# aniketntnu/WordDiffusion

Measured on AMD Instinct MI355X. Metric: denoised 64x256 word images/sec (1000-step DDPM), whole job, higher is better.
Workload: dtype bf16x3; 1 GPU; BASELINE configs[1]: batch 64 per GPU of 64x256 crops = [64,4,8,32] latents, 1000-step DDPM (999 executed steps), base unet.py UNetModel (320 ch, mult (1,1), 4 heads, 339 writers), random-init synthetic weights; variant=base, batch_per_gpu=64, noise_steps=1000, executed_steps_per_image=999, precision=split-bf16 MFMA x3, fp32 accumulate (<=1e-4 of the fp32 reference), output_finite=True

## Files before the change

worddiffusion_amd/csrc/wd_gemmq.hip:

```cpp
#include "wd_gemm_epi.h"
#include "wd_gemm_priv.h"

namespace {

constexpr int QNT = 512;
constexpr int QBM = 64, QBN = 80;
constexpr int QLDE = QBN + 4;
constexpr uint32_t Q_OOB = 0x80000000u;

typedef __attribute__((ext_vector_type(4))) unsigned q_u32x4;

__device__ __forceinline__ int q_lds_off(int row, int ch) { return row * 128 + ((ch ^ ((row >> 1) & 7)) << 4); }

__global__ void __launch_bounds__(QNT, 1) wd_gemmq_kernel(const wd_gemm_args a, const int nbn, const int nbm, const int nchp) {
#if defined(__HIP_DEVICE_COMPILE__)
    extern __shared__ __attribute__((aligned(16))) char smem[];
    const int ntile = nbn * nbm;
    int wg;
    {
        const int bid = blockIdx.x;
        const int q = ntile >> 3, r = ntile & 7, xcd = bid & 7, loc = bid >> 3;
        wg = (xcd < r ? xcd * (q + 1) : r * (q + 1) + (xcd - r) * q) + loc;
    }
    const int bn_i = wg % nbn, bm_i = wg / nbn;
    const int m0 = bm_i * QBM, n0 = bn_i * QBN;
    const int tid = threadIdx.x;
    const int lane = tid & 63;
    const int wave = __builtin_amdgcn_readfirstlane(tid >> 6);
    const int l15 = lane & 15, lq = lane >> 4;

    const int W = a.src[0].ntaps == 9 ? a.slab_rows : 0;
    const int wsh = W ? __builtin_ctz(W) : 0;
    const int ST = (W && a.src[0].hw_src == 4 * a.hw_out) ? 2 : 1;
    const int Ws = W * ST, wss = wsh + ST - 1;
    const int Hs = W ? (a.hw_out >> wsh) * ST : 0;
    const int TR = W ? QBM >> wsh : 0;
    const int NR = W ? (TR - 1) * ST + 3 : 0;
    const int SW = Ws + 2;
    const int bsm = m0 / a.hw_out;
    const int y0 = W ? (m0 - bsm * a.hw_out) >> wsh : 0;

    auto make_srd = [](const void* p) {
        return __builtin_amdgcn_make_buffer_rsrc(const_cast<void*>(p), 0, 0x7FFFFFF0, 0x00020000);
    };
    const __amdgpu_buffer_rsrc_t srd_w_hi = make_srd(a.w_hi), srd_w_lo = make_srd(a.w_lo);

    const int nct = a.n >> 4;
    const uint32_t b_voff = (uint32_t)((n0 >> 4) * 1024 + lane * 16);
    const uint32_t kstep_bytes = (uint32_t)nct * 1024u;
    auto load_b = [&](bf16x8 (&fb)[5][2], const int kabs, const bool live) {
        const uint32_t so = live ? (uint32_t)kabs * kstep_bytes : 0u;
        const uint32_t vo = live ? b_voff : Q_OOB;
#pragma unroll
        for (int t = 0; t < 5; ++t)
#pragma unroll
            for (int p = 0; p < 2; ++p)
                fb[t][p] = __builtin_bit_cast(bf16x8, __builtin_amdgcn_raw_buffer_load_b128(p ? srd_w_lo : srd_w_hi, vo + t * 1024, so, 0));
    };
    f32x4 acc[4][5];
#pragma unroll
    for (int i = 0; i < 4; ++i)
#pragma unroll
        for (int t = 0; t < 5; ++t)
#pragma unroll
            for (int r = 0; r < 4; ++r) acc[i][t][r] = 0.0f;
    auto mfma_step = [&](const char* base, const int cpl, const int (&rb)[4], const int shift0, const int lm, const int half,
                         const bf16x8 (&fb)[5][2], const int skip) {
        const int ach = half * 4 + lq;
        const int shift = shift0 + lm * l15 - l15;
        bf16x8 xa[2][2];
        {
            const int ao = q_lds_off(rb[0] + shift + l15, ach);
            xa[0][0] = *reinterpret_cast<const bf16x8*>(base + ao);
            xa[0][1] = *reinterpret_cast<const bf16x8*>(base + cpl + ao);
        }
#pragma unroll
        for (int i = 0; i < 4; ++i) {
            if (i < 3) {
                const int ao = q_lds_off(rb[i + 1] + shift + l15, ach);
                xa[(i + 1) & 1][0] = *reinterpret_cast<const bf16x8*>(base + ao);
                xa[(i + 1) & 1][1] = *reinterpret_cast<const bf16x8*>(base + cpl + ao);
            }
            if (skip & (1 << i)) continue;
#pragma unroll
            for (int t = 0; t < 5; ++t) {
                acc[i][t] = __builtin_amdgcn_mfma_f32_16x16x32_bf16(xa[i & 1][1], fb[t][0], acc[i][t], 0, 0, 0);
                acc[i][t] = __builtin_amdgcn_mfma_f32_16x16x32_bf16(xa[i & 1][0], fb[t][1], acc[i][t], 0, 0, 0);
                acc[i][t] = __builtin_amdgcn_mfma_f32_16x16x32_bf16(xa[i & 1][0], fb[t][0], acc[i][t], 0, 0, 0);
            }
        }
    };
#ifdef WD_Q_STAMPS
    unsigned long long* qst = (a.dbg & 0x100) && a.ws && blockIdx.x == 0 ? reinterpret_cast<unsigned long long*>(a.ws) + wave * 8 : nullptr;
#define Q_STAMP(i) if (qst && lane == 0) qst[i] = __builtin_amdgcn_s_memtime()
#else
#define Q_STAMP(i)
#endif
    Q_STAMP(0);
    bf16x8 xb[5][2], yb[5][2];
    bool first_pass = true;

    auto run_source = [&](const wd_src& q, const bool conv, const int kbase) {
        const int cpt = q.c >> 6;
        const int slr = conv ? NR * SW : QBM;
        const int cpl = slr * 128, chb = 2 * cpl;
        const int pchunks = min(conv ? 5 : 8, (140 * 1024) / chb);
        const int kpc = conv ? 18 : 2;
        const int ntok = conv ? NR * Ws : QBM;
        const int lm = conv ? ST : 1;
        const __amdgpu_buffer_rsrc_t srd_a_hi = make_srd(q.hi), srd_a_lo = make_srd(q.lo);
        int rb[4];
        int skm0 = 0, skm2 = 0;
#pragma unroll
        for (int i = 0; i < 4; ++i) {
            const int p = 16 * i;
            rb[i] = conv ? ST * (p >> wsh) * SW + ST * (p & (W - 1)) : p;
            if (conv) {
                const int ys = ST * (y0 + (p >> wsh)) - 1;
                if (ys < 0) skm0 |= 1 << i;
                if (ys + 2 >= Hs) skm2 |= 1 << i;
            }
        }
        for (int c_lo = 0; c_lo < cpt; c_lo += pchunks) {
            const int nch = min(pchunks, cpt - c_lo);
            const int nks = kpc * nch;
            if (!first_pass) __syncthreads();
            first_pass = false;
            auto kabs_of = [&](const int c, const int r) {
                return kbase + (conv ? 2 * ((r >> 1) * cpt + c_lo + c) + (r & 1) : 2 * (c_lo + c) + r);
            };
            auto advance = [&](int& c, int& r) {
                if (conv) {
                    r += 8;
                    const bool wrap = r >= 18;
                    r = __builtin_amdgcn_readfirstlane(wrap ? r - 18 : r);
                    c = __builtin_amdgcn_readfirstlane(wrap ? c + 1 : c);
                } else {
                    c += 4;
                }
            };
            auto skip_of = [&](const int r) {
                if (!conv) return 0;
                const int ky = (r >> 1) / 3;
                return __builtin_amdgcn_readfirstlane(ky == 0 ? skm0 : ky == 2 ? skm2 : 0);
            };
            auto shift_of = [&](const int r) {
                if (!conv) return 0;
                const int tap = r >> 1, ky = tap / 3;
                return ky * SW + (tap - 3 * ky);
            };
            int nc = conv ? 0 : wave >> 1, nr = conv ? wave : wave & 1;
            int cc = nc, cr = nr;
            load_b(xb, kabs_of(nc, nr), kpc * nc + nr < nks);
            advance(nc, nr);
            if (conv) {
                for (int i = tid; i < nch * 2 * NR * 2 * 8; i += QNT) {
                    const int pc = i & 7, side = (i >> 3) & 1;
                    int rest = i >> 4;
                    const int ry = rest % NR;
                    rest /= NR;
                    const int pl = rest & 1, ch = rest >> 1;
                    const int row = ry * SW + (side ? SW - 1 : 0);
                    *reinterpret_cast<q_u32x4*>(smem + ch * chb + pl * cpl + row * 128 + pc * 16) = q_u32x4{0u, 0u, 0u, 0u};
                }
            }
            const int nitems = nch * ntok * 8;
            for (int i0 = 0; i0 < nitems; i0 += 8 * QNT) {
                q_u32x4 v[2][8];
                int dst[8];
#pragma unroll
                for (int k = 0; k < 8; ++k) {
                    const int i = i0 + k * QNT + tid;
                    const int pc = i & 7;
                    const int rest = i >> 3;
                    const int chl = rest / ntok, tq = rest - chl * ntok;
                    int grow, srow;
                    bool ok = i < nitems;
                    if (conv) {
                        const int ry = tq >> wss, x = tq & (Ws - 1);
                        const int gy = ST * y0 - 1 + ry;
                        ok = ok && gy >= 0 && gy < Hs;
                        grow = bsm * q.hw_src + gy * Ws + x;
                        srow = ry * SW + x + 1;
                    } else {
                        grow = m0 + tq;
                        srow = tq;
                    }
                    const uint32_t vo = ok ? (uint32_t)grow * (uint32_t)(q.ld * 2) + (uint32_t)((c_lo + chl) * 128 + pc * 16) : Q_OOB;
                    v[0][k] = __builtin_amdgcn_raw_buffer_load_b128(srd_a_hi, vo, 0, 0);
                    v[1][k] = __builtin_amdgcn_raw_buffer_load_b128(srd_a_lo, vo, 0, 0);
                    dst[k] = i < nitems ? chl * chb + q_lds_off(srow, pc) : -1;
                }
#pragma unroll
                for (int k = 0; k < 8; ++k)
                    if (dst[k] >= 0) {
                        *reinterpret_cast<q_u32x4*>(smem + dst[k]) = v[0][k];
                        *reinterpret_cast<q_u32x4*>(smem + dst[k] + cpl) = v[1][k];
                    }
            }
            __syncthreads();
            Q_STAMP(1);
            for (int ks = wave; ks < nks; ks += 16) {
                load_b(yb, kabs_of(nc, nr), kpc * nc + nr < nks);
                advance(nc, nr);
                __builtin_amdgcn_sched_barrier(0);
                mfma_step(smem + cc * chb, cpl, rb, shift_of(cr), lm, cr & 1, xb, skip_of(cr));
                __builtin_amdgcn_sched_barrier(0);
                advance(cc, cr);
                load_b(xb, kabs_of(nc, nr), kpc * nc + nr < nks);
                advance(nc, nr);
                __builtin_amdgcn_sched_barrier(0);
                if (kpc * cc + cr < nks) mfma_step(smem + cc * chb, cpl, rb, shift_of(cr), lm, cr & 1, yb, skip_of(cr));
                __builtin_amdgcn_sched_barrier(0);
                advance(cc, cr);
            }
        }
    };
    const bool conv0 = a.src[0].ntaps == 9;
    run_source(a.src[0], conv0, 0);
    if (a.nsrc > 1) run_source(a.src[1], false, 2 * a.src[0].ntaps * (a.src[0].c >> 6));

    Q_STAMP(4);
    __syncthreads();
    Q_STAMP(5);
    constexpr int IMG = QBM * QLDE;
    constexpr int CLD = QBM + 4;
    constexpr int PIMG = QBN * CLD;
    float* res = reinterpret_cast<float*>(smem);
    float* part = res + IMG;
    auto pcol = [&](float* b, const int i, const int t) -> f32x4* {
        return reinterpret_cast<f32x4*>(b + (t * 16 + l15) * CLD + i * 16 + 4 * lq);
    };
    if (wave >= 4) {
        float* b = part + (wave - 4) * PIMG;
#pragma unroll
        for (int i = 0; i < 4; ++i)
#pragma unroll
            for (int t = 0; t < 5; ++t) *pcol(b, i, t) = acc[i][t];
    }
    __syncthreads();
    if (wave < 4) {
        float* b = part + wave * PIMG;
#pragma unroll
        for (int i = 0; i < 4; ++i)
#pragma unroll
            for (int t = 0; t < 5; ++t) {
                acc[i][t] += *pcol(b, i, t);
                *pcol(b, i, t) = acc[i][t];
            }
    }
    __syncthreads();
    for (int e = tid; e < QBN * (QBM / 4); e += QNT) {
        const int col = e >> 4, r4 = (e & 15) * 4;
        const float* p = part + col * CLD + r4;
        f32x4 v = *reinterpret_cast<const f32x4*>(p);
        v += *reinterpret_cast<const f32x4*>(p + PIMG);
        v += *reinterpret_cast<const f32x4*>(p + 2 * PIMG);
        v += *reinterpret_cast<const f32x4*>(p + 3 * PIMG);
#pragma unroll
        for (int r = 0; r < 4; ++r) res[(r4 + r) * QLDE + col] = v[r];
    }
    __syncthreads();
    float* buf = res;
    Q_STAMP(6);
    if (a.gn_gamma) wd_gn_tile<QBN, QNT, false>(a, buf, buf + IMG, m0, n0, tid);
    else wd_epilogue_tail<QBM, QBN, QNT>(a, buf, m0, n0, tid, 0);
    Q_STAMP(7);
#endif
}

}

bool wd_gemmq_applies(const wd_gemm_args& a) {
    const int W = a.slab_rows;
    if (!(a.w_layout == 3 && a.tile == 64080 && !a.a32 && !a.ln_gamma && a.npass == 3 && a.ksplit <= 1 && a.m % 64 == 0 && a.n % QBN == 0 &&
          a.act == WD_ACT_NONE && !a.resid_rows && a.nsrc >= 1 && a.nsrc <= 2))
        return false;
    for (int s = 0; s < a.nsrc; ++s) {
        const wd_src& q = a.src[s];
        if (!q.hi || !q.lo || q.c % 64 || (q.ld & 7)) return false;
        const bool conv = s == 0 && q.ntaps == 9 && q.gather && a.hw_out == 64 &&
                          (((W == 16 || W == 32) && q.hw_src == 64) || (W == 16 && q.hw_src == 256));
        const bool ident = q.ntaps == 1 && !q.gather;
        if (!conv && !ident) return false;
    }
    return true;
}

int wd_gemmq_launch(const wd_gemm_args& a, hipStream_t st) {
    const int loop_smem = 140 * 1024;
    const int red_smem = (QBM * QLDE + 4 * QBN * (QBM + 4)) * 4 + WD_STAT_SCRATCH;
    const int smem = loop_smem > red_smem ? loop_smem : red_smem;
    const int nchp = 0;
    static int attr_max = 0;
    if (smem > attr_max) {
        if (hipFuncSetAttribute(reinterpret_cast<const void*>(&wd_gemmq_kernel), hipFuncAttributeMaxDynamicSharedMemorySize, smem) != hipSuccess)
            return WD_ELAUNCH;
        attr_max = smem;
    }
    const int nbn = a.n / QBN, nbm = a.m / QBM;
    {
        WdLaunchScope scope(WD_CLS_GEMM_Q, st, 2.0 * (double)a.m * (double)a.n * (double)a.ktot);
        hipLaunchKernelGGL(wd_gemmq_kernel, dim3(nbn * nbm), dim3(QNT), smem, st, a, nbn, nbm, nchp);
    }
    return wd_check_launch();
}
```

worddiffusion_amd/csrc/wd_ff.hip:

```cpp
#include "wd_gemm_epi.h"

namespace {

constexpr int FNT = 512;
constexpr int FBM = 64;
constexpr int FC = 320;
constexpr int FCH = 128;
constexpr int FRING = 6;
constexpr int F_MAX_INNER = 2048;
constexpr int FGRP = 30;
constexpr uint32_t F_OOB = 0x80000000u;

typedef __attribute__((ext_vector_type(4))) unsigned f_u32x4;

__device__ __forceinline__ int f_lds_off(int row, int ch) { return row * 128 + ((ch ^ ((row >> 1) & 7)) << 4); }

template <int NPASS, bool PROJ, bool FRONT>
__global__ void __launch_bounds__(FNT, 1) wd_ff_kernel(const wd_ff_args a) {
#if defined(__HIP_DEVICE_COMPILE__)
    static_assert(!FRONT || (NPASS == 3 && PROJ), "the transformer front needs split-bf16 operands and the proj_out tail");
    constexpr int NPL = (NPASS == 1) ? 1 : 2;
    constexpr int SLAB = 2 * FBM * 128;
    constexpr int A_BYTES = 5 * SLAB;
    constexpr int H_BYTES = 2 * SLAB;
    extern __shared__ __attribute__((aligned(16))) char smem[];
    char* s_a = smem;
    char* s_h = smem + A_BYTES;
    float* s_b1 = reinterpret_cast<float*>(smem + A_BYTES + 2 * H_BYTES);

    const int m0 = blockIdx.x * FBM;
    const int tid = threadIdx.x;
    const int lane = tid & 63;
    const int wave = __builtin_amdgcn_readfirstlane(tid >> 6);
    const int kh = wave >> 2, cg = wave & 3;
    const int l15 = lane & 15, lq = lane >> 4;
    const int nchunk = a.inner / FCH;

    auto make_srd = [](const wd_bf16* p) {
        return __builtin_amdgcn_make_buffer_rsrc(const_cast<wd_bf16*>(p), 0, 0x7FFFFFF0, 0x00020000);
    };
    const __amdgpu_buffer_rsrc_t srd1_hi = make_srd(a.w1_hi), srd1_lo = make_srd(a.w1_lo ? a.w1_lo : a.w1_hi);
    const __amdgpu_buffer_rsrc_t srd2_hi = make_srd(a.w2_hi), srd2_lo = make_srd(a.w2_lo ? a.w2_lo : a.w2_hi);
    const __amdgpu_buffer_rsrc_t srd3_hi = make_srd(PROJ ? a.w3_hi : a.w2_hi), srd3_lo = make_srd(PROJ ? (a.w3_lo ? a.w3_lo : a.w3_hi) : a.w2_hi);
    const uint32_t lane16 = lane * 16;
    const int nct1 = (2 * a.inner) >> 4;

    bf16x8 ring[FRING][NPL];
    auto issue = [&](const int slot, const int g, const int j) {
        const bool live = j < nchunk;
        const uint32_t vo = live ? lane16 : F_OOB;
        if (PROJ && g < FRING) {
            const uint32_t so3 = (uint32_t)(((2 * (g / 5) + kh) * (FC / 16) + 5 * cg + g % 5) * 1024);
            const uint32_t so1 = (uint32_t)(((g >> 1) * nct1 + 2 * (j * 8 + wave) + (g & 1)) * 1024);
            const uint32_t so = live ? so1 : so3;
#pragma unroll
            for (int p = 0; p < NPL; ++p) {
                const __amdgpu_buffer_rsrc_t srd = live ? (p ? srd1_lo : srd1_hi) : (p ? srd3_lo : srd3_hi);
                ring[slot][p] = __builtin_bit_cast(bf16x8, __builtin_amdgcn_raw_buffer_load_b128(srd, lane16, so, 0));
            }
        } else if (g < 20) {
            const uint32_t so = (uint32_t)(((g >> 1) * nct1 + 2 * (j * 8 + wave) + (g & 1)) * 1024);
#pragma unroll
            for (int p = 0; p < NPL; ++p)
                ring[slot][p] = __builtin_bit_cast(bf16x8, __builtin_amdgcn_raw_buffer_load_b128(p ? srd1_lo : srd1_hi, vo, live ? so : 0u, 0));
        } else {
            const int q = (g - 20) / 5, t = (g - 20) % 5;
            const uint32_t so = (uint32_t)(((4 * j + 2 * kh + q) * (FC / 16) + 5 * cg + t) * 1024);
#pragma unroll
            for (int p = 0; p < NPL; ++p)
                ring[slot][p] = __builtin_bit_cast(bf16x8, __builtin_amdgcn_raw_buffer_load_b128(p ? srd2_lo : srd2_hi, vo, live ? so : 0u, 0));
        }
    };
    f32x4 acc2[4][5];
    bf16x8 xa[4][NPL];
    auto read_frags = [&](const char* slab_base, const int half) {
        const int ch = half * 4 + lq;
#pragma unroll
        for (int i = 0; i < 4; ++i) {
            const int ao = f_lds_off(i * 16 + l15, ch);
#pragma unroll
            for (int p = 0; p < NPL; ++p) xa[i][p] = *reinterpret_cast<const bf16x8*>(slab_base + p * (FBM * 128) + ao);
        }
    };
    auto mfma12 = [&](f32x4 (&acc)[4], const bf16x8 (&w)[NPL]) {
#pragma unroll
        for (int i = 0; i < 4; ++i) {
            if (NPL == 2) {
                acc[i] = __builtin_amdgcn_mfma_f32_16x16x32_bf16(xa[i][NPL - 1], w[0], acc[i], 0, 0, 0);
                acc[i] = __builtin_amdgcn_mfma_f32_16x16x32_bf16(xa[i][0], w[NPL - 1], acc[i], 0, 0, 0);
            }
            acc[i] = __builtin_amdgcn_mfma_f32_16x16x32_bf16(xa[i][0], w[0], acc[i], 0, 0, 0);
        }
    };
    constexpr int LDE = FC + 4;
    float* ep = reinterpret_cast<float*>(smem);
    auto ksum_to_image = [&]() {
        for (int hh = 0; hh < 2; ++hh) {
            if (kh == hh) {
#pragma unroll
                for (int i = 0; i < 4; ++i)
#pragma unroll
                    for (int t = 0; t < 5; ++t)
#pragma unroll
                        for (int r = 0; r < 4; ++r) {
                            float* pe = ep + (i * 16 + 4 * lq + r) * LDE + cg * 80 + t * 16 + l15;
                            *pe = (hh == 0) ? acc2[i][t][r] : *pe + acc2[i][t][r];
                        }
            }
            __syncthreads();
        }
    };

    if constexpr (FRONT) {
        constexpr int SP = 65, PP = 72, KS32 = FC / 32;
        const int b = m0 / a.hw;
        const int HJ = a.heads * a.L;
        char* fr = s_h + 4096;
        float* s_aff = reinterpret_cast<float*>(fr);
        float* sS = reinterpret_cast<float*>(fr);
        wd_bf16* sP = reinterpret_cast<wd_bf16*>(fr + FBM * SP * 4);
        {
            const int ngp = FC / a.gn_pcpg, ratio = a.gn_cpg / a.gn_pcpg;
            for (int c = tid; c < FC; c += FNT) {
                const int g = c / a.gn_cpg;
                double su = 0.0, sq = 0.0;
                for (int k = 0; k < ratio; ++k)
                    for (int ck = 0; ck < a.gn_nchunk; ++ck) {
                        const double* pp = a.gn_part + (((long)b * a.gn_nchunk + ck) * ngp + g * ratio + k) * 2;
                        su += pp[0];
                        sq += pp[1];
                    }
                const double n = (double)a.hw * a.gn_cpg;
                const double mu = su / n;
                double var = sq / n - mu * mu;
                if (var < 0.0) var = 0.0;
                const float rstd = (float)(1.0 / sqrt(var + (double)a.gn_eps));
                const float sc = rstd * a.gn_gamma[c];
                s_aff[2 * c] = sc;
                s_aff[2 * c + 1] = a.gn_beta[c] - (float)mu * sc;
            }
            for (int e = tid; e < FBM * PP; e += FNT) reinterpret_cast<uint32_t*>(sP)[e] = 0u;
        }
        const int arow = tid >> 3, ach = tid & 7;
        float4 xv[5][2];
        {
            const float* xrow = a.x_in + (long)(m0 + arow) * a.x_in_ld + ach * 8;
#pragma unroll
            for (int sl = 0; sl < 5; ++sl) {
                xv[sl][0] = *reinterpret_cast<const float4*>(xrow + sl * 64);
                xv[sl][1] = *reinterpret_cast<const float4*>(xrow + sl * 64 + 4);
            }
        }
        const __amdgpu_buffer_rsrc_t srdp_hi = make_srd(a.pi_hi), srdp_lo = make_srd(a.pi_lo);
        auto issue_pi = [&](const int slot, const int g) {
            const uint32_t so = (uint32_t)(((2 * (g / 5) + kh) * (FC / 16) + 5 * cg + g % 5) * 1024);
#pragma unroll
            for (int p = 0; p < NPL; ++p)
                ring[slot][p] = __builtin_bit_cast(bf16x8, __builtin_amdgcn_raw_buffer_load_b128(p ? srdp_lo : srdp_hi, lane16, so, 0));
        };
#pragma unroll
        for (int g = 0; g < FRING; ++g) issue_pi(g, g);
        __syncthreads();
#pragma unroll
        for (int sl = 0; sl < 5; ++sl) {
            const float4* tab = reinterpret_cast<const float4*>(s_aff + 2 * (sl * 64 + ach * 8));
            const float4 t0 = tab[0], t1 = tab[1], t2 = tab[2], t3 = tab[3];
            const float4 x0 = xv[sl][0], x1 = xv[sl][1];
            float4 y0, y1;
            y0.x = x0.x * t0.x + t0.y; y0.y = x0.y * t0.z + t0.w; y0.z = x0.z * t1.x + t1.y; y0.w = x0.w * t1.z + t1.w;
            y1.x = x1.x * t2.x + t2.y; y1.y = x1.y * t2.z + t2.w; y1.z = x1.z * t3.x + t3.y; y1.w = x1.w * t3.z + t3.w;
            uint2 h0, l0, h1, l1;
            wd_split4(y0, h0, l0);
            wd_split4(y1, h1, l1);
            char* dst = s_a + sl * SLAB + f_lds_off(arow, ach);
            *reinterpret_cast<f_u32x4*>(dst) = f_u32x4{h0.x, h0.y, h1.x, h1.y};
            *reinterpret_cast<f_u32x4*>(dst + FBM * 128) = f_u32x4{l0.x, l0.y, l1.x, l1.y};
        }
        __syncthreads();
#pragma unroll
        for (int i = 0; i < 4; ++i)
#pragma unroll
            for (int t = 0; t < 5; ++t)
#pragma unroll
                for (int r = 0; r < 4; ++r) acc2[i][t][r] = 0.0f;
#pragma unroll
        for (int g = 0; g < 25; ++g) {
            const int q = g / 5, t = g % 5;
            if (t == 0) read_frags(s_a + q * SLAB, kh);
            {
                f32x4 col[4] = {acc2[0][t], acc2[1][t], acc2[2][t], acc2[3][t]};
                mfma12(col, ring[g % FRING]);
#pragma unroll
                for (int i = 0; i < 4; ++i) acc2[i][t] = col[i];
            }
            if (g + FRING < 25) issue_pi(g % FRING, g + FRING);
            __builtin_amdgcn_sched_barrier(0);
        }
        __syncthreads();
        ksum_to_image();
        float4 xr[2][5];
#pragma unroll
        for (int pp = 0; pp < 2; ++pp)
#pragma unroll
            for (int i = 0; i < 5; ++i) {
                const int n = (l15 + 16 * i) * 4, row = wave * 8 + pp * 4 + lq;
                const float4 v = *reinterpret_cast<const float4*>(ep + row * LDE + n);
                const float4 bx = *reinterpret_cast<const float4*>(a.pi_b + n);
                xr[pp][i] = make_float4(v.x + bx.x, v.y + bx.y, v.z + bx.z, v.w + bx.w);
            }
        __syncthreads();
        auto ln_rows = [&](const float* gamma, const float* beta) {
#pragma unroll
            for (int pp = 0; pp < 2; ++pp) {
                const int row = wave * 8 + pp * 4 + lq;
                float s = 0.f;
#pragma unroll
                for (int i = 0; i < 5; ++i) s += (xr[pp][i].x + xr[pp][i].y) + (xr[pp][i].z + xr[pp][i].w);
                const float mean = wd_row16_sum(s) / (float)FC;
                float q = 0.f;
#pragma unroll
                for (int i = 0; i < 5; ++i) {
                    const float a0 = xr[pp][i].x - mean, a1 = xr[pp][i].y - mean, a2 = xr[pp][i].z - mean, a3 = xr[pp][i].w - mean;
                    q += (a0 * a0 + a1 * a1) + (a2 * a2 + a3 * a3);
                }
                const float rstd = 1.0f / sqrtf(wd_row16_sum(q) / (float)FC + a.ln_eps);
#pragma unroll
                for (int i = 0; i < 5; ++i) {
                    const int n = (l15 + 16 * i) * 4;
                    const float4 ga = *reinterpret_cast<const float4*>(gamma + n);
                    const float4 be = *reinterpret_cast<const float4*>(beta + n);
                    const float4 x = xr[pp][i];
                    float4 o;
                    o.x = (x.x - mean) * rstd * ga.x + be.x; o.y = (x.y - mean) * rstd * ga.y + be.y;
                    o.z = (x.z - mean) * rstd * ga.z + be.z; o.w = (x.w - mean) * rstd * ga.w + be.w;
                    uint2 hi, lo;
                    wd_split4(o, hi, lo);
                    char* d = s_a + (n >> 6) * SLAB + f_lds_off(row, (n & 63) >> 3) + (n & 7) * 2;
                    *reinterpret_cast<uint2*>(d) = hi;
                    *reinterpret_cast<uint2*>(d + FBM * 128) = lo;
                }
            }
        };
        const int ht = wave & 3, rp = wave >> 2;
        const long pq = 64L * FC;
#pragma unroll
        for (int ps = 0; ps < 2; ++ps) {
            const wd_bf16* mq = ps == 0 ? a.mq_a : a.mq_b;
            const wd_bf16* mot = ps == 0 ? a.mot_a : a.mot_b;
            const float* xb = ps == 0 ? a.xb_a : a.xb_b;
            ln_rows(a.ln2_gamma, a.ln2_beta);
            __builtin_amdgcn_sched_barrier(0);
            bf16x8 bh[KS32], bl[KS32];
            {
                const __amdgpu_buffer_rsrc_t rq = __builtin_amdgcn_make_buffer_rsrc(const_cast<wd_bf16*>(mq + (long)b * 2 * pq), 0,
                                                                                    (int)(2 * pq * 2), 0x00020000);
                const uint32_t vo = ht * 16 + l15 < HJ ? lane16 : F_OOB;
#pragma unroll
                for (int ks = 0; ks < KS32; ++ks) {
                    bh[ks] = __builtin_bit_cast(bf16x8, __builtin_amdgcn_raw_buffer_load_b128(rq, vo, (uint32_t)((ht * KS32 + ks) << 10), 0));
                    bl[ks] = __builtin_bit_cast(bf16x8, __builtin_amdgcn_raw_buffer_load_b128(rq, vo, (uint32_t)(((ht * KS32 + ks) << 10) + pq * 2), 0));
                }
            }
            __syncthreads();
            if (ht * 16 < HJ) {
                f32x4 a_lh[2], a_hl[2], a_hh[2];
#pragma unroll
                for (int ri = 0; ri < 2; ++ri)
#pragma unroll
                    for (int r = 0; r < 4; ++r) a_lh[ri][r] = a_hl[ri][r] = a_hh[ri][r] = 0.f;
#pragma unroll
                for (int ks = 0; ks < KS32; ++ks)
#pragma unroll
                    for (int ri = 0; ri < 2; ++ri) {
                        const char* ap = s_a + (ks >> 1) * SLAB + f_lds_off((2 * rp + ri) * 16 + l15, (ks & 1) * 4 + lq);
                        const bf16x8 ah = *reinterpret_cast<const bf16x8*>(ap);
                        const bf16x8 al = *reinterpret_cast<const bf16x8*>(ap + FBM * 128);
                        a_lh[ri] = __builtin_amdgcn_mfma_f32_16x16x32_bf16(al, bh[ks], a_lh[ri], 0, 0, 0);
                        a_hl[ri] = __builtin_amdgcn_mfma_f32_16x16x32_bf16(ah, bl[ks], a_hl[ri], 0, 0, 0);
                        a_hh[ri] = __builtin_amdgcn_mfma_f32_16x16x32_bf16(ah, bh[ks], a_hh[ri], 0, 0, 0);
                    }
#pragma unroll
                for (int ri = 0; ri < 2; ++ri)
#pragma unroll
                    for (int r = 0; r < 4; ++r)
                        sS[((2 * rp + ri) * 16 + 4 * lq + r) * SP + ht * 16 + l15] = (a_lh[ri][r] + a_hl[ri][r]) + a_hh[ri][r];
            }
            __builtin_amdgcn_sched_barrier(0);
            bf16x8 mh[2][5], ml[2][5];
            {
                const __amdgpu_buffer_rsrc_t rm = __builtin_amdgcn_make_buffer_rsrc(const_cast<wd_bf16*>(mot + (long)b * 2 * pq), 0,
                                                                                    (int)(2 * pq * 2), 0x00020000);
#pragma unroll
                for (int ks = 0; ks < 2; ++ks) {
                    const uint32_t vo = ks * 32 + lq * 8 < HJ ? lane16 : F_OOB;
#pragma unroll
                    for (int t = 0; t < 5; ++t) {
                        const uint32_t so = (uint32_t)((((5 * cg + t) * 2 + ks) << 10));
                        mh[ks][t] = __builtin_bit_cast(bf16x8, __builtin_amdgcn_raw_buffer_load_b128(rm, vo, so, 0));
                        ml[ks][t] = __builtin_bit_cast(bf16x8, __builtin_amdgcn_raw_buffer_load_b128(rm, vo, so + (uint32_t)(pq * 2), 0));
                    }
                }
            }
            __syncthreads();
            for (int idx = tid; idx < FBM * a.heads; idx += FNT) {
                const int t = idx / a.heads, h = idx - t * a.heads;
                const float* pr = sS + t * SP + h * a.L;
                wd_bf16* ph = sP + t * PP + h * a.L;
                float mx = -3.4e38f;
                for (int j = 0; j < a.L; ++j) mx = fmaxf(mx, pr[j]);
                float sum = 0.f;
                for (int j = 0; j < a.L; ++j) sum += __expf(pr[j] - mx);
                const float inv = __fdividef(1.f, sum);
                for (int j = 0; j < a.L; ++j) {
                    uint32_t hi, lo;
                    wd_split1(__expf(pr[j] - mx) * inv, hi, lo);
                    ph[j] = (wd_bf16)hi;
                    ph[FBM * PP + j] = (wd_bf16)lo;
                }
            }
            __syncthreads();
            {
                f32x4 o[2][5];
#pragma unroll
                for (int ri = 0; ri < 2; ++ri)
#pragma unroll
                    for (int t = 0; t < 5; ++t)
#pragma unroll
                        for (int r = 0; r < 4; ++r) o[ri][t][r] = 0.f;
#pragma unroll
                for (int ks = 0; ks < 2; ++ks)
#pragma unroll
                    for (int ri = 0; ri < 2; ++ri) {
                        const wd_bf16* ap = sP + ((2 * rp + ri) * 16 + l15) * PP + lq * 8 + ks * 32;
                        const bf16x8 ah = *reinterpret_cast<const bf16x8*>(ap);
                        const bf16x8 al = *reinterpret_cast<const bf16x8*>(ap + FBM * PP);
#pragma unroll
                        for (int t = 0; t < 5; ++t) o[ri][t] = __builtin_amdgcn_mfma_f32_16x16x32_bf16(al, mh[ks][t], o[ri][t], 0, 0, 0);
#pragma unroll
                        for (int t = 0; t < 5; ++t) o[ri][t] = __builtin_amdgcn_mfma_f32_16x16x32_bf16(ah, ml[ks][t], o[ri][t], 0, 0, 0);
#pragma unroll
                        for (int t = 0; t < 5; ++t) o[ri][t] = __builtin_amdgcn_mfma_f32_16x16x32_bf16(ah, mh[ks][t], o[ri][t], 0, 0, 0);
                    }
#pragma unroll
                for (int ri = 0; ri < 2; ++ri)
#pragma unroll
                    for (int t = 0; t < 5; ++t)
#pragma unroll
                        for (int r = 0; r < 4; ++r) ep[((2 * rp + ri) * 16 + 4 * lq + r) * LDE + (5 * cg + t) * 16 + l15] = o[ri][t][r];
            }
            __syncthreads();
#pragma unroll
            for (int pp = 0; pp < 2; ++pp)
#pragma unroll
                for (int i = 0; i < 5; ++i) {
                    const int n = (l15 + 16 * i) * 4, row = wave * 8 + pp * 4 + lq;
                    const float4 bi = *reinterpret_cast<const float4*>(xb + n);
                    const float4 at = *reinterpret_cast<const float4*>(ep + row * LDE + n);
                    const float4 x = xr[pp][i];
                    xr[pp][i] = make_float4(at.x + bi.x + x.x, at.y + bi.y + x.y, at.z + bi.z + x.z, at.w + bi.w + x.w);
                }
            __syncthreads();
        }
#pragma unroll
        for (int pp = 0; pp < 2; ++pp)
#pragma unroll
            for (int i = 0; i < 5; ++i)
                *reinterpret_cast<float4*>(a.tok2 + (long)(m0 + wave * 8 + pp * 4 + lq) * FC + (l15 + 16 * i) * 4) = xr[pp][i];
        ln_rows(a.ln3_gamma, a.ln3_beta);
        for (int i = tid; i < 2 * a.inner; i += FNT) s_b1[i] = a.b1 ? a.b1[i] : 0.0f;
        __builtin_amdgcn_sched_barrier(0);
#pragma unroll
        for (int g = 0; g < FRING; ++g) issue(g, g, 0);
    } else {
#pragma unroll
    for (int g = 0; g < FRING; ++g) issue(g, g, 0);

    {
        const __amdgpu_buffer_rsrc_t sx_hi = make_srd(a.x_hi), sx_lo = make_srd(a.x_lo ? a.x_lo : a.x_hi);
        const int arow = tid >> 3, ach = tid & 7;
        const uint32_t vo = (m0 + arow < a.m) ? (uint32_t)(m0 + arow) * (uint32_t)(a.x_ld * 2) + (uint32_t)(ach * 16) : F_OOB;
        f_u32x4 v[5][NPL];
#pragma unroll
        for (int sl = 0; sl < 5; ++sl)
#pragma unroll
            for (int p = 0; p < NPL; ++p) v[sl][p] = __builtin_amdgcn_raw_buffer_load_b128(p ? sx_lo : sx_hi, vo, sl * 128, 0);
        const int dst = f_lds_off(arow, ach);
#pragma unroll
        for (int sl = 0; sl < 5; ++sl)
#pragma unroll
            for (int p = 0; p < NPL; ++p) *reinterpret_cast<f_u32x4*>(s_a + sl * SLAB + p * (FBM * 128) + dst) = v[sl][p];
        for (int i = tid; i < 2 * a.inner; i += FNT) s_b1[i] = a.b1 ? a.b1[i] : 0.0f;
    }
    }
    __syncthreads();

#pragma unroll
    for (int i = 0; i < 4; ++i)
#pragma unroll
        for (int t = 0; t < 5; ++t)
#pragma unroll
            for (int r = 0; r < 4; ++r) acc2[i][t][r] = 0.0f;

    for (int j = 0; j < nchunk; ++j) {
        char* hbuf = s_h + (j & 1) * H_BYTES;
        f32x4 ax[4], ag[4];
#pragma unroll
        for (int i = 0; i < 4; ++i)
#pragma unroll
            for (int r = 0; r < 4; ++r) {
                ax[i][r] = 0.0f;
                ag[i][r] = 0.0f;
            }
#pragma unroll
        for (int g = 0; g < 20; ++g) {
            if ((g & 1) == 0) read_frags(s_a + (g >> 2) * SLAB, (g >> 1) & 1);
            if (g & 1) mfma12(ag, ring[g % FRING]);
            else mfma12(ax, ring[g % FRING]);
            if (g + FRING < FGRP) issue(g % FRING, g + FRING, j);
            else issue(g % FRING, g + FRING - FGRP, j + 1);
            __builtin_amdgcn_sched_barrier(0);
        }
        {
            const int hcol = (j * 8 + wave) * 32 + l15;
            const float bx = s_b1[hcol], bg = s_b1[hcol + 16];
            const int slab = wave >> 2, ch = (wave & 3) * 2 + (l15 >> 3), e = (l15 & 7) * 2;
#pragma unroll
            for (int i = 0; i < 4; ++i)
#pragma unroll
                for (int r = 0; r < 4; ++r) {
                    const float h = (ax[i][r] + bx) * wd_gelu_erf(ag[i][r] + bg);
                    uint32_t hb, lb;
                    wd_split1(h, hb, lb);
                    char* p = hbuf + slab * SLAB + f_lds_off(i * 16 + lq * 4 + r, ch) + e;
                    *reinterpret_cast<unsigned short*>(p) = (unsigned short)hb;
                    if (NPL == 2) *reinterpret_cast<unsigned short*>(p + FBM * 128) = (unsigned short)lb;
                }
        }
        __syncthreads();
#pragma unroll
        for (int g = 20; g < FGRP; ++g) {
            const int q = (g - 20) / 5, t = (g - 20) % 5;
            if (t == 0) read_frags(hbuf + kh * SLAB, q);
            {
                f32x4 col[4] = {acc2[0][t], acc2[1][t], acc2[2][t], acc2[3][t]};
                mfma12(col, ring[g % FRING]);
#pragma unroll
                for (int i = 0; i < 4; ++i) acc2[i][t] = col[i];
            }
            if (g + FRING < FGRP) issue(g % FRING, g + FRING, j);
            else issue(g % FRING, g + FRING - FGRP, j + 1);
            __builtin_amdgcn_sched_barrier(0);
        }
    }

    __syncthreads();
    ksum_to_image();
    wd_gemm_args e = {};
    e.m = a.m;
    e.n = FC;
    e.hw_out = a.hw_out > 0 ? a.hw_out : 1;
    e.act = WD_ACT_NONE;
    e.out_f32 = a.out_f32;
    e.out_ld = a.out_ld;
    e.out_hi = a.out_hi;
    e.out_lo = a.out_lo;
    e.out_pl_ld = a.out_pl_ld;
    e.ksplit = 1;
    e.stat_part = a.stat_part;
    e.stat_cpg = a.stat_cpg;
    if constexpr (!PROJ) {
        e.bias = a.b2;
        e.resid = a.resid;
        e.resid_ld = a.resid_ld;
        wd_epilogue_from_image<FBM, FC, FNT>(e, ep, m0, 0, tid);
    } else {
        constexpr int ROWB = LDE * 4;
        const float* resid = FRONT ? a.tok2 : a.resid;
        const int resid_ld = FRONT ? FC : a.resid_ld;
        if (FRONT) asm volatile("s_waitcnt vmcnt(0)" ::: "memory");
        {
            float4 v[10];
#pragma unroll
            for (int it = 0; it < 10; ++it) {
                const int idx = it * 64 + lane, row = wave * 8 + idx / 80, c = (idx % 80) * 4;
                const int m = m0 + row;
                float4 x = *reinterpret_cast<const float4*>(ep + row * LDE + c);
                if (a.b2) {
                    const float4 q = *reinterpret_cast<const float4*>(a.b2 + c);
                    x.x += q.x; x.y += q.y; x.z += q.z; x.w += q.w;
                }
                if (resid && m < a.m) {
                    const float4 q = *reinterpret_cast<const float4*>(resid + (long)m * resid_ld + c);
                    x.x += q.x; x.y += q.y; x.z += q.z; x.w += q.w;
                }
                v[it] = x;
            }
            asm volatile("s_waitcnt lgkmcnt(0)" ::: "memory");
            __builtin_amdgcn_sched_barrier(0);
#pragma unroll
            for (int it = 0; it < 10; ++it) {
                const int idx = it * 64 + lane, row = wave * 8 + idx / 80, c = (idx % 80) * 4;
                uint2 hh, ll;
                wd_split4(v[it], hh, ll);
                char* rowp = reinterpret_cast<char*>(ep) + row * ROWB;
                *reinterpret_cast<uint2*>(rowp + c * 2) = hh;
                if (NPL == 2) *reinterpret_cast<uint2*>(rowp + 640 + c * 2) = ll;
            }
        }
        __syncthreads();
#pragma unroll
        for (int i = 0; i < 4; ++i)
#pragma unroll
            for (int t = 0; t < 5; ++t)
#pragma unroll
                for (int r = 0; r < 4; ++r) acc2[i][t][r] = 0.0f;
#pragma unroll
        for (int g = 0; g < 25; ++g) {
            const int q = g / 5, t = g % 5;
            if (t == 0) {
                const int ks = 2 * q + kh;
#pragma unroll
                for (int i = 0; i < 4; ++i) {
                    const char* rp = reinterpret_cast<const char*>(ep) + (i * 16 + l15) * ROWB + (ks * 4 + lq) * 16;
#pragma unroll
                    for (int p = 0; p < NPL; ++p) xa[i][p] = *reinterpret_cast<const bf16x8*>(rp + p * 640);
// ... 85 lines not shown
```

Measured before the change: 34.15 images/s.

## Stream identity GEMM A operands from registers and overlap conv LDS fill with MFMA

Identity (1x1) sources no longer stage A tiles through LDS. Each wave loads its A fragments directly from global memory with double-buffered registers, which removes the fill pass and barriers. For the 3x3 conv source, only the first channel chunk is filled before compute starts. The remaining chunks are loaded in small batches interleaved with the first MFMA steps, followed by one barrier. The LDS budget grows to 160KB, and the direct global A loads may be less coalesced and less reused than the shared LDS tile was.

Measured after the change: 34.24 images/s (median of 6 runs). About the same (+0.2%).

```diff
diff --git a/worddiffusion_amd/csrc/wd_gemmq.hip b/worddiffusion_amd/csrc/wd_gemmq.hip
--- a/worddiffusion_amd/csrc/wd_gemmq.hip
+++ b/worddiffusion_amd/csrc/wd_gemmq.hip
@@ -6,6 +6,7 @@
 constexpr int QNT = 512;
 constexpr int QBM = 64, QBN = 80;
 constexpr int QLDE = QBN + 4;
+constexpr int Q_LOOP_SMEM = 160 * 1024;
 constexpr uint32_t Q_OOB = 0x80000000u;
 
 typedef __attribute__((ext_vector_type(4))) unsigned q_u32x4;
@@ -100,125 +101,183 @@
     bf16x8 xb[5][2], yb[5][2];
     bool first_pass = true;
 
-    auto run_source = [&](const wd_src& q, const bool conv, const int kbase) {
+    auto run_ident = [&](const wd_src& q, const int kbase) {
+        const int nks = 2 * (q.c >> 6);
+        const __amdgpu_buffer_rsrc_t srd_a_hi = make_srd(q.hi), srd_a_lo = make_srd(q.lo);
+        const uint32_t rowb = (uint32_t)q.ld * 2u;
+        const uint32_t a_voff = (uint32_t)(m0 + l15) * rowb + (uint32_t)(lq * 16);
+        auto load_a = [&](bf16x8 (&fa)[4][2], const int ks, const bool live) {
+            const uint32_t so = live ? (uint32_t)ks * 64u : 0u;
+#pragma unroll
+            for (int i = 0; i < 4; ++i) {
+                const uint32_t vo = live ? a_voff + (uint32_t)(16 * i) * rowb : Q_OOB;
+#pragma unroll
+                for (int p = 0; p < 2; ++p)
+                    fa[i][p] = __builtin_bit_cast(bf16x8, __builtin_amdgcn_raw_buffer_load_b128(p ? srd_a_lo : srd_a_hi, vo, so, 0));
+            }
+        };
+        auto mfma_regs = [&](const bf16x8 (&fa)[4][2], const bf16x8 (&fb)[5][2]) {
+#pragma unroll
+            for (int i = 0; i < 4; ++i)
+#pragma unroll
+                for (int t = 0; t < 5; ++t) {
+                    acc[i][t] = __builtin_amdgcn_mfma_f32_16x16x32_bf16(fa[i][1], fb[t][0], acc[i][t], 0, 0, 0);
+                    acc[i][t] = __builtin_amdgcn_mfma_f32_16x16x32_bf16(fa[i][0], fb[t][1], acc[i][t], 0, 0, 0);
+                    acc[i][t] = __builtin_amdgcn_mfma_f32_16x16x32_bf16(fa[i][0], fb[t][0], acc[i][t], 0, 0, 0);
+                }
+        };
+        bf16x8 xa[4][2], ya[4][2];
+        load_b(xb, kbase + wave, wave < nks);
+        load_a(xa, wave, wave < nks);
+        for (int ks = wave; ks < nks; ks += 16) {
+            load_b(yb, kbase + ks + 8, ks + 8 < nks);
+            load_a(ya, ks + 8, ks + 8 < nks);
+            __builtin_amdgcn_sched_barrier(0);
+            mfma_regs(xa, xb);
+            __builtin_amdgcn_sched_barrier(0);
+            load_b(xb, kbase + ks + 16, ks + 16 < nks);
+            load_a(xa, ks + 16, ks + 16 < nks);
+            __builtin_amdgcn_sched_barrier(0);
+            if (ks + 8 < nks) mfma_regs(ya, yb);
+            __builtin_amdgcn_sched_barrier(0);
+        }
+    };
+
+    constexpr int QR = 2;
+    auto run_source = [&](const wd_src& q, const int kbase) {
         const int cpt = q.c >> 6;
-        const int slr = conv ? NR * SW : QBM;
-        const int cpl = slr * 128, chb = 2 * cpl;
-        const int pchunks = min(conv ? 5 : 8, (140 * 1024) / chb);
-        const int kpc = conv ? 18 : 2;
-        const int ntok = conv ? NR * Ws : QBM;
-        const int lm = conv ? ST : 1;
+        const int cpl = NR * SW * 128, chb = 2 * cpl;
+        const int pchunks = min(5, Q_LOOP_SMEM / chb);
+        constexpr int kpc = 18;
+        const int ntok = NR * Ws;
         const __amdgpu_buffer_rsrc_t srd_a_hi = make_srd(q.hi), srd_a_lo = make_srd(q.lo);
         int rb[4];
         int skm0 = 0, skm2 = 0;
 #pragma unroll
         for (int i = 0; i < 4; ++i) {
             const int p = 16 * i;
-            rb[i] = conv ? ST * (p >> wsh) * SW + ST * (p & (W - 1)) : p;
-            if (conv) {
-                const int ys = ST * (y0 + (p >> wsh)) - 1;
-                if (ys < 0) skm0 |= 1 << i;
-                if (ys + 2 >= Hs) skm2 |= 1 << i;
-            }
+            rb[i] = ST * (p >> wsh) * SW + ST * (p & (W - 1));
+            const int ys = ST * (y0 + (p >> wsh)) - 1;
+            if (ys < 0) skm0 |= 1 << i;
+            if (ys + 2 >= Hs) skm2 |= 1 << i;
         }
         for (int c_lo = 0; c_lo < cpt; c_lo += pchunks) {
             const int nch = min(pchunks, cpt - c_lo);
             const int nks = kpc * nch;
             if (!first_pass) __syncthreads();
             first_pass = false;
-            auto kabs_of = [&](const int c, const int r) {
-                return kbase + (conv ? 2 * ((r >> 1) * cpt + c_lo + c) + (r & 1) : 2 * (c_lo + c) + r);
-            };
+            auto kabs_of = [&](const int c, const int r) { return kbase + 2 * ((r >> 1) * cpt + c_lo + c) + (r & 1); };
             auto advance = [&](int& c, int& r) {
-                if (conv) {
-                    r += 8;
-                    const bool wrap = r >= 18;
-                    r = __builtin_amdgcn_readfirstlane(wrap ? r - 18 : r);
-                    c = __builtin_amdgcn_readfirstlane(wrap ? c + 1 : c);
-                } else {
-                    c += 4;
-                }
+                r += 8;
+                const bool wrap = r >= 18;
+                r = __builtin_amdgcn_readfirstlane(wrap ? r - 18 : r);
+                c = __builtin_amdgcn_readfirstlane(wrap ? c + 1 : c);
             };
             auto skip_of = [&](const int r) {
-                if (!conv) return 0;
                 const int ky = (r >> 1) / 3;
                 return __builtin_amdgcn_readfirstlane(ky == 0 ? skm0 : ky == 2 ? skm2 : 0);
             };
             auto shift_of = [&](const int r) {
-                if (!conv) return 0;
                 const int tap = r >> 1, ky = tap / 3;
                 return ky * SW + (tap - 3 * ky);
             };
-            int nc = conv ? 0 : wave >> 1, nr = conv ? wave : wave & 1;
+            int nc = 0, nr = wave;
             int cc = nc, cr = nr;
             load_b(xb, kabs_of(nc, nr), kpc * nc + nr < nks);
             advance(nc, nr);
-            if (conv) {
-                for (int i = tid; i < nch * 2 * NR * 2 * 8; i += QNT) {
-                    const int pc = i & 7, side = (i >> 3) & 1;
-                    int rest = i >> 4;
-                    const int ry = rest % NR;
-                    rest /= NR;
-                    const int pl = rest & 1, ch = rest >> 1;
-                    const int row = ry * SW + (side ? SW - 1 : 0);
-                    *reinterpret_cast<q_u32x4*>(smem + ch * chb + pl * cpl + row * 128 + pc * 16) = q_u32x4{0u, 0u, 0u, 0u};
-                }
-            }
-            const int nitems = nch * ntok * 8;
-            for (int i0 = 0; i0 < nitems; i0 += 8 * QNT) {
-                q_u32x4 v[2][8];
-                int dst[8];
-#pragma unroll
-                for (int k = 0; k < 8; ++k) {
+            for (int i = tid; i < nch * 2 * NR * 2 * 8; i += QNT) {
+                const int pc = i & 7, side = (i >> 3) & 1;
+                int rest = i >> 4;
+                const int ry = rest % NR;
+                rest /= NR;
+                const int pl = rest & 1, ch = rest >> 1;
+                const int row = ry * SW + (side ? SW - 1 : 0);
+                *reinterpret_cast<q_u32x4*>(smem + ch * chb + pl * cpl + row * 128 + pc * 16) = q_u32x4{0u, 0u, 0u, 0u};
+            }
+            const int nitems = nch * ntok * 8, n0 = ntok * 8;
+            auto fill_load = [&](q_u32x4 (&v)[2][QR], const int i0, const int iend) {
+#pragma unroll
+                for (int k = 0; k < QR; ++k) {
                     const int i = i0 + k * QNT + tid;
                     const int pc = i & 7;
                     const int rest = i >> 3;
                     const int chl = rest / ntok, tq = rest - chl * ntok;
-                    int grow, srow;
-                    bool ok = i < nitems;
-                    if (conv) {
-                        const int ry = tq >> wss, x = tq & (Ws - 1);
-                        const int gy = ST * y0 - 1 + ry;
-                        ok = ok && gy >= 0 && gy < Hs;
-                        grow = bsm * q.hw_src + gy * Ws + x;
-                        srow = ry * SW + x + 1;
-                    } else {
-                        grow = m0 + tq;
-                        srow = tq;
-                    }
+                    const int ry = tq >> wss, x = tq & (Ws - 1);
+                    const int gy = ST * y0 - 1 + ry;
+                    const bool ok = i < iend && gy >= 0 && gy < Hs;
+                    const int grow = bsm * q.hw_src + gy * Ws + x;
                     const uint32_t vo = ok ? (uint32_t)grow * (uint32_t)(q.ld * 2) + (uint32_t)((c_lo + chl) * 128 + pc * 16) : Q_OOB;
                     v[0][k] = __builtin_amdgcn_raw_buffer_load_b128(srd_a_hi, vo, 0, 0);
                     v[1][k] = __builtin_amdgcn_raw_buffer_load_b128(srd_a_lo, vo, 0, 0);
-                    dst[k] = i < nitems ? chl * chb + q_lds_off(srow, pc) : -1;
                 }
-#pragma unroll
-                for (int k = 0; k < 8; ++k)
-                    if (dst[k] >= 0) {
-                        *reinterpret_cast<q_u32x4*>(smem + dst[k]) = v[0][k];
-                        *reinterpret_cast<q_u32x4*>(smem + dst[k] + cpl) = v[1][k];
+            };
+            auto fill_store = [&](const q_u32x4 (&v)[2][QR], const int i0, const int iend) {
+#pragma unroll
+                for (int k = 0; k < QR; ++k) {
+                    const int i = i0 + k * QNT + tid;
+                    if (i < iend) {
+                        const int pc = i & 7;
+                        const int rest = i >> 3;
+                        const int chl = rest / ntok, tq = rest - chl * ntok;
+                        const int ry = tq >> wss, x = tq & (Ws - 1);
+                        const int dst = chl * chb + q_lds_off(ry * SW + x + 1, pc);
+                        *reinterpret_cast<q_u32x4*>(smem + dst) = v[0][k];
+                        *reinterpret_cast<q_u32x4*>(smem + dst + cpl) = v[1][k];
                     }
+                }
+            };
+            q_u32x4 fv[2][QR];
+            for (int i0 = 0; i0 < n0; i0 += QR * QNT) {
+                fill_load(fv, i0, n0);
+                fill_store(fv, i0, n0);
             }
             __syncthreads();
             Q_STAMP(1);
-            for (int ks = wave; ks < nks; ks += 16) {
+            auto step_x = [&]() {
                 load_b(yb, kabs_of(nc, nr), kpc * nc + nr < nks);
                 advance(nc, nr);
                 __builtin_amdgcn_sched_barrier(0);
-                mfma_step(smem + cc * chb, cpl, rb, shift_of(cr), lm, cr & 1, xb, skip_of(cr));
+                mfma_step(smem + cc * chb, cpl, rb, shift_of(cr), ST, cr & 1, xb, skip_of(cr));
                 __builtin_amdgcn_sched_barrier(0);
                 advance(cc, cr);
+            };
+            auto step_y = [&]() {
                 load_b(xb, kabs_of(nc, nr), kpc * nc + nr < nks);
                 advance(nc, nr);
                 __builtin_amdgcn_sched_barrier(0);
-                if (kpc * cc + cr < nks) mfma_step(smem + cc * chb, cpl, rb, shift_of(cr), lm, cr & 1, yb, skip_of(cr));
+                if (kpc * cc + cr < nks) mfma_step(smem + cc * chb, cpl, rb, shift_of(cr), ST, cr & 1, yb, skip_of(cr));
                 __builtin_amdgcn_sched_barrier(0);
                 advance(cc, cr);
+            };
+            int ks = wave;
+            if (nch > 1) {
+                int i0 = n0;
+                fill_load(fv, i0, nitems);
+                __builtin_amdgcn_sched_barrier(0);
+                step_x();
+                fill_store(fv, i0, nitems);
+                i0 += QR * QNT;
+                fill_load(fv, i0, nitems);
+                __builtin_amdgcn_sched_barrier(0);
+                step_y();
+                fill_store(fv, i0, nitems);
+                for (i0 += QR * QNT; i0 < nitems; i0 += QR * QNT) {
+                    fill_load(fv, i0, nitems);
+                    fill_store(fv, i0, nitems);
+                }
+                __syncthreads();
+                ks += 16;
+            }
+            for (; ks < nks; ks += 16) {
+                step_x();
+                step_y();
             }
         }
     };
     const bool conv0 = a.src[0].ntaps == 9;
-    run_source(a.src[0], conv0, 0);
-    if (a.nsrc > 1) run_source(a.src[1], false, 2 * a.src[0].ntaps * (a.src[0].c >> 6));
+    if (conv0) run_source(a.src[0], 0);
+    else run_ident(a.src[0], 0);
+    if (a.nsrc > 1) run_ident(a.src[1], 2 * a.src[0].ntaps * (a.src[0].c >> 6));
 
     Q_STAMP(4);
     __syncthreads();
@@ -288,7 +347,7 @@
 }
 
 int wd_gemmq_launch(const wd_gemm_args& a, hipStream_t st) {
-    const int loop_smem = 140 * 1024;
+    const int loop_smem = Q_LOOP_SMEM;
     const int red_smem = (QBM * QLDE + 4 * QBN * (QBM + 4)) * 4 + WD_STAT_SCRATCH;
     const int smem = loop_smem > red_smem ? loop_smem : red_smem;
     const int nchp = 0;
```

## Prefetch front-path vectors, GN partials and next-stage weights earlier in fused FF kernel

Applied to the files above, without the earlier changes.

In the transformer-front path of the fused feed-forward kernel, the GroupNorm partial sums, bias/LayerNorm parameter vectors and b1 are now loaded into registers up front and staged into LDS once, instead of being read from global memory inside later loops. The mq weight fragments for each cross-attention pass and the first FF weight ring slots are issued earlier, during the previous stage's MFMA work, so their latency overlaps compute. This raises register pressure and uses more LDS, and it relies on a static LDS map assertion holding.

New measurement: 34.18 images/s before, 34.63 images/s after, median of 6. 1.01x the previous value.

```diff
diff --git a/worddiffusion_amd/csrc/wd_ff.hip b/worddiffusion_amd/csrc/wd_ff.hip
--- a/worddiffusion_amd/csrc/wd_ff.hip
+++ b/worddiffusion_amd/csrc/wd_ff.hip
@@ -119,28 +119,35 @@
         float* s_aff = reinterpret_cast<float*>(fr);
         float* sS = reinterpret_cast<float*>(fr);
         wd_bf16* sP = reinterpret_cast<wd_bf16*>(fr + FBM * SP * 4);
-        {
-            const int ngp = FC / a.gn_pcpg, ratio = a.gn_cpg / a.gn_pcpg;
-            for (int c = tid; c < FC; c += FNT) {
-                const int g = c / a.gn_cpg;
-                double su = 0.0, sq = 0.0;
-                for (int k = 0; k < ratio; ++k)
-                    for (int ck = 0; ck < a.gn_nchunk; ++ck) {
-                        const double* pp = a.gn_part + (((long)b * a.gn_nchunk + ck) * ngp + g * ratio + k) * 2;
-                        su += pp[0];
-                        sq += pp[1];
-                    }
-                const double n = (double)a.hw * a.gn_cpg;
-                const double mu = su / n;
-                double var = sq / n - mu * mu;
-                if (var < 0.0) var = 0.0;
-                const float rstd = (float)(1.0 / sqrt(var + (double)a.gn_eps));
-                const float sc = rstd * a.gn_gamma[c];
-                s_aff[2 * c] = sc;
-                s_aff[2 * c + 1] = a.gn_beta[c] - (float)mu * sc;
-            }
-            for (int e = tid; e < FBM * PP; e += FNT) reinterpret_cast<uint32_t*>(sP)[e] = 0u;
-        }
+        float* s_vec = reinterpret_cast<float*>(s_h + 40960);
+        const float* s_pib = s_vec;
+        const float *s_ln2g = s_vec + FC, *s_ln2b = s_vec + 2 * FC, *s_ln3g = s_vec + 3 * FC, *s_ln3b = s_vec + 4 * FC;
+        const float *s_xba = s_vec + 5 * FC, *s_xbb = s_vec + 6 * FC;
+        constexpr int NVEC = 7, V4 = FC / 4;
+        static_assert(4096 + FBM * SP * 4 + 2 * FBM * PP * 2 <= 40960 && 40960 + NVEC * FC * 4 <= 2 * H_BYTES, "front LDS map");
+        auto vec_src = [&](const int i) {
+            const int v = i / V4;
+            const float* p = v == 0 ? a.pi_b : v == 1 ? a.ln2_gamma : v == 2 ? a.ln2_beta : v == 3 ? a.ln3_gamma : v == 4 ? a.ln3_beta
+                           : v == 5 ? a.xb_a : a.xb_b;
+            return reinterpret_cast<const float4*>(p) + (i - v * V4);
+        };
+        const int ngp = FC / a.gn_pcpg, ratio = a.gn_cpg / a.gn_pcpg;
+        const int gc = tid < FC ? tid : FC - 1;
+        const int gg = gc / a.gn_cpg;
+        const int npart = ratio * a.gn_nchunk;
+        auto part_ptr = [&](const int i) {
+            const int k = i / a.gn_nchunk, ck = i - k * a.gn_nchunk;
+            return a.gn_part + (((long)b * a.gn_nchunk + ck) * ngp + gg * ratio + k) * 2;
+        };
+        constexpr int GB = 4;
+        double gsu[GB], gsq[GB];
+#pragma unroll
+        for (int i = 0; i < GB; ++i) {
+            const double* pp = part_ptr(i < npart ? i : 0);
+            gsu[i] = pp[0];
+            gsq[i] = pp[1];
+        }
+        const float gn_ga = a.gn_gamma[gc], gn_be = a.gn_beta[gc];
         const int arow = tid >> 3, ach = tid & 7;
         float4 xv[5][2];
         {
@@ -151,6 +158,19 @@
                 xv[sl][1] = *reinterpret_cast<const float4*>(xrow + sl * 64 + 4);
             }
         }
+        const float4 sv0 = *vec_src(tid);
+        const float4 sv1 = *vec_src(tid < NVEC * V4 - FNT ? FNT + tid : NVEC * V4 - 1);
+        constexpr int NB1 = 2 * F_MAX_INNER / FNT;
+        float b1v[NB1];
+        {
+            const float* b1p = a.b1 ? a.b1 : a.pi_b;
+#pragma unroll
+            for (int k = 0; k < NB1; ++k) {
+                const bool in = a.b1 && k * FNT + tid < 2 * a.inner;
+                const float v = b1p[in ? k * FNT + tid : 0];
+                b1v[k] = in ? v : 0.0f;
+            }
+        }
         const __amdgpu_buffer_rsrc_t srdp_hi = make_srd(a.pi_hi), srdp_lo = make_srd(a.pi_lo);
         auto issue_pi = [&](const int slot, const int g) {
             const uint32_t so = (uint32_t)(((2 * (g / 5) + kh) * (FC / 16) + 5 * cg + g % 5) * 1024);
@@ -160,6 +180,37 @@
         };
 #pragma unroll
         for (int g = 0; g < FRING; ++g) issue_pi(g, g);
+        __builtin_amdgcn_sched_barrier(0);
+        {
+            double su = 0.0, sq = 0.0;
+#pragma unroll
+            for (int i = 0; i < GB; ++i)
+                if (i < npart) {
+                    su += gsu[i];
+                    sq += gsq[i];
+                }
+            for (int i = GB; i < npart; ++i) {
+                const double* pp = part_ptr(i);
+                su += pp[0];
+                sq += pp[1];
+            }
+            const double n = (double)a.hw * a.gn_cpg;
+            const double mu = su / n;
+            double var = sq / n - mu * mu;
+            if (var < 0.0) var = 0.0;
+            const float rstd = (float)(1.0 / sqrt(var + (double)a.gn_eps));
+            const float sc = rstd * gn_ga;
+            if (tid < FC) {
+                s_aff[2 * tid] = sc;
+                s_aff[2 * tid + 1] = gn_be - (float)mu * sc;
+            }
+            for (int e = tid; e < FBM * PP; e += FNT) reinterpret_cast<uint32_t*>(sP)[e] = 0u;
+            reinterpret_cast<float4*>(s_vec)[tid] = sv0;
+            if (tid < NVEC * V4 - FNT) reinterpret_cast<float4*>(s_vec)[FNT + tid] = sv1;
+#pragma unroll
+            for (int k = 0; k < NB1; ++k)
+                if (k * FNT + tid < 2 * a.inner) s_b1[k * FNT + tid] = b1v[k];
+        }
         __syncthreads();
 #pragma unroll
         for (int sl = 0; sl < 5; ++sl) {
@@ -196,6 +247,22 @@
             if (g + FRING < 25) issue_pi(g % FRING, g + FRING);
             __builtin_amdgcn_sched_barrier(0);
         }
+        const int ht = wave & 3, rp = wave >> 2;
+        const long pq = 64L * FC;
+        bf16x8 bh[KS32], bl[KS32];
+        constexpr int FEARLY = 4;
+        auto issue_mq = [&](const wd_bf16* mq) {
+            const __amdgpu_buffer_rsrc_t rq = __builtin_amdgcn_make_buffer_rsrc(const_cast<wd_bf16*>(mq + (long)b * 2 * pq), 0,
+                                                                                (int)(2 * pq * 2), 0x00020000);
+            const uint32_t vo = ht * 16 + l15 < HJ ? lane16 : F_OOB;
+#pragma unroll
+            for (int ks = 0; ks < KS32; ++ks) {
+                bh[ks] = __builtin_bit_cast(bf16x8, __builtin_amdgcn_raw_buffer_load_b128(rq, vo, (uint32_t)((ht * KS32 + ks) << 10), 0));
+                bl[ks] = __builtin_bit_cast(bf16x8, __builtin_amdgcn_raw_buffer_load_b128(rq, vo, (uint32_t)(((ht * KS32 + ks) << 10) + pq * 2), 0));
+            }
+        };
+        issue_mq(a.mq_a);
+        __builtin_amdgcn_sched_barrier(0);
         __syncthreads();
         ksum_to_image();
         float4 xr[2][5];
@@ -205,7 +272,7 @@
             for (int i = 0; i < 5; ++i) {
                 const int n = (l15 + 16 * i) * 4, row = wave * 8 + pp * 4 + lq;
                 const float4 v = *reinterpret_cast<const float4*>(ep + row * LDE + n);
-                const float4 bx = *reinterpret_cast<const float4*>(a.pi_b + n);
+                const float4 bx = *reinterpret_cast<const float4*>(s_pib + n);
                 xr[pp][i] = make_float4(v.x + bx.x, v.y + bx.y, v.z + bx.z, v.w + bx.w);
             }
         __syncthreads();
@@ -241,26 +308,17 @@
                 }
             }
         };
-        const int ht = wave & 3, rp = wave >> 2;
-        const long pq = 64L * FC;
 #pragma unroll
         for (int ps = 0; ps < 2; ++ps) {
-            const wd_bf16* mq = ps == 0 ? a.mq_a : a.mq_b;
             const wd_bf16* mot = ps == 0 ? a.mot_a : a.mot_b;
-            const float* xb = ps == 0 ? a.xb_a : a.xb_b;
-            ln_rows(a.ln2_gamma, a.ln2_beta);
+            const float* xb = ps == 0 ? s_xba : s_xbb;
+            if (ps == 1) {
+#pragma unroll
+                for (int g = 0; g < FEARLY; ++g) issue(g, g, 0);
+                __builtin_amdgcn_sched_barrier(0);
+            }
+            ln_rows(s_ln2g, s_ln2b);
             __builtin_amdgcn_sched_barrier(0);
-            bf16x8 bh[KS32], bl[KS32];
-            {
-                const __amdgpu_buffer_rsrc_t rq = __builtin_amdgcn_make_buffer_rsrc(const_cast<wd_bf16*>(mq + (long)b * 2 * pq), 0,
-                                                                                    (int)(2 * pq * 2), 0x00020000);
-                const uint32_t vo = ht * 16 + l15 < HJ ? lane16 : F_OOB;
-#pragma unroll
-                for (int ks = 0; ks < KS32; ++ks) {
-                    bh[ks] = __builtin_bit_cast(bf16x8, __builtin_amdgcn_raw_buffer_load_b128(rq, vo, (uint32_t)((ht * KS32 + ks) << 10), 0));
-                    bl[ks] = __builtin_bit_cast(bf16x8, __builtin_amdgcn_raw_buffer_load_b128(rq, vo, (uint32_t)(((ht * KS32 + ks) << 10) + pq * 2), 0));
-                }
-            }
             __syncthreads();
             if (ht * 16 < HJ) {
                 f32x4 a_lh[2], a_hl[2], a_hh[2];
@@ -341,6 +399,14 @@
 #pragma unroll
                         for (int t = 0; t < 5; ++t) o[ri][t] = __builtin_amdgcn_mfma_f32_16x16x32_bf16(ah, mh[ks][t], o[ri][t], 0, 0, 0);
                     }
+                __builtin_amdgcn_sched_barrier(0);
+                if (ps == 0) {
+                    issue_mq(a.mq_b);
+                } else {
+#pragma unroll
+                    for (int g = FEARLY; g < FRING; ++g) issue(g, g, 0);
+                }
+                __builtin_amdgcn_sched_barrier(0);
 #pragma unroll
                 for (int ri = 0; ri < 2; ++ri)
 #pragma unroll
@@ -366,11 +432,7 @@
 #pragma unroll
             for (int i = 0; i < 5; ++i)
                 *reinterpret_cast<float4*>(a.tok2 + (long)(m0 + wave * 8 + pp * 4 + lq) * FC + (l15 + 16 * i) * 4) = xr[pp][i];
-        ln_rows(a.ln3_gamma, a.ln3_beta);
-        for (int i = tid; i < 2 * a.inner; i += FNT) s_b1[i] = a.b1 ? a.b1[i] : 0.0f;
-        __builtin_amdgcn_sched_barrier(0);
-#pragma unroll
-        for (int g = 0; g < FRING; ++g) issue(g, g, 0);
+        ln_rows(s_ln3g, s_ln3b);
     } else {
 #pragma unroll
     for (int g = 0; g < FRING; ++g) issue(g, g, 0);
```
